# Yukun-Huang/DreamWaltz-G

Hardware: AMD Instinct MI355X
Metric: SDS steps/sec @512^2, 100k Gaussians, SD1.5+ControlNet; raster Mpix/s vs HBM roofline (higher is better)
Workload: dtype f32x

## Files before the change

dreamwaltz-g_amd/csrc/gemm.hip:

```cpp
#include "dwg_common.h"
#include "dwg_prof_internal.h"
#include "../../include/dwg_gemm.h"
#include <cstdlib>
#include <type_traits>

#if defined(DWG_GEMM_X_TU)
#include "dwg_xfmt.h"
typedef _Float16 HT;
#define DWG_DTYPE_HALF DWG_DTYPE_F32X
#define DWG_MFMA16(a, b, c) __builtin_amdgcn_mfma_f32_32x32x16_f16(a, b, c, 0, 0, 0)
#define DWG_HALF_NAME "f32x"
#elif defined(DWG_GEMM_F16_TU)
typedef _Float16 HT;
#define DWG_DTYPE_HALF DWG_DTYPE_F16
#define DWG_MFMA16(a, b, c) __builtin_amdgcn_mfma_f32_32x32x16_f16(a, b, c, 0, 0, 0)
#define DWG_HALF_NAME "f16"
#else
typedef __bf16 HT;
#define DWG_DTYPE_HALF DWG_DTYPE_BF16
#define DWG_MFMA16(a, b, c) __builtin_amdgcn_mfma_f32_32x32x16_bf16(a, b, c, 0, 0, 0)
#define DWG_HALF_NAME "bf16"
#endif

namespace {

typedef __attribute__((ext_vector_type(8))) HT bf16x8;
typedef __attribute__((ext_vector_type(16))) float f32x16;

struct ConvP {
    int enabled, Cin, Hin, Win, Hout, Wout, KH, KW, stride, pad_t, pad_l, dil;
    int up;
    int cin1;
    const void* A2;
};

struct GemmP {
    const void* A; const void* B; void* C; const void* bias; const void* residual;
    int M, N, K;
    long long sam, sak, sbn, sbk, ldc, ldr;
    int nb2;
    long long bA1, bA2, bB1, bB2, bC1, bC2, bR1, bR2;
    int act; float alpha;
    int out_bf16, res_bf16, bias_per_row, splitk, accumulate;
    float* ws;
    int bias_row_div;
    long long bias_ld;
    ConvP conv;
};

__device__ __forceinline__ float bf2f(HT x) { return (float)x; }
__device__ __forceinline__ HT f2bf(float x) { return (HT)x; }

struct bf16x4_t { HT v[4]; };
#ifdef DWG_GEMM_X_TU
__device__ __forceinline__ float ld_half1(const void* base, long long i) { return dwg_x_get1(base, i); }
__device__ __forceinline__ void st_half1(void* base, long long i, float v) { dwg_x_put1(base, i, v); }
__device__ __forceinline__ void ld_half4(const void* base, long long i, float (&v)[4]) { dwg_x_get4(base, i, v); }
__device__ __forceinline__ void st_half4(void* base, long long i, const float (&v)[4]) { dwg_x_put4(base, i, v); }
#else
__device__ __forceinline__ float ld_half1(const void* base, long long i) { return bf2f(reinterpret_cast<const HT*>(base)[i]); }
__device__ __forceinline__ void st_half1(void* base, long long i, float v) { reinterpret_cast<HT*>(base)[i] = f2bf(v); }
__device__ __forceinline__ void ld_half4(const void* base, long long i, float (&v)[4]) {
    const bf16x4_t r = *reinterpret_cast<const bf16x4_t*>(reinterpret_cast<const HT*>(base) + i);
#pragma unroll
    for (int e = 0; e < 4; e++) v[e] = bf2f(r.v[e]);
}
__device__ __forceinline__ void st_half4(void* base, long long i, const float (&v)[4]) {
    bf16x4_t o;
#pragma unroll
    for (int e = 0; e < 4; e++) o.v[e] = f2bf(v[e]);
    *reinterpret_cast<bf16x4_t*>(reinterpret_cast<HT*>(base) + i) = o;
}
#endif

template <bool LIGHT = false>
__device__ __forceinline__ float apply_act(float v, int act) {
    if constexpr (LIGHT) return act == 3 ? v / (1.f + __expf(-v)) : v;
    switch (act) {
        case 1: return v > 0.f ? v : 0.f;
        case 2: return v > 0.f ? v : 0.01f * v;
        case 3: return v / (1.f + __expf(-v));
        case 4: return 0.5f * v * (1.f + erff(v * 0.70710678118654752f));
        case 5: return 1.f / (1.f + __expf(-v));
        default: return v;
    }
}

// ... 840 lines not shown
    double f = 2.0 * p.M * p.N * p.K * batch;
#ifdef DWG_GEMM_X_TU
    f *= 0.5;
#endif
    if (p.conv.enabled && p.conv.dil > 1) f /= (double)(p.conv.dil * p.conv.dil);
    return f;
}

template <int BN, int AKIND>
static void launch_glds(const GemmP& p, int batch, hipStream_t stream, const char* name) {
    constexpr int S = (BN == 64 && AKIND != 1) ? 3 : 2;
    size_t lds = (size_t)S * (128 + BN) * 128;
    static bool attr_set = false;
    if (!attr_set) {
        hipFuncSetAttribute(reinterpret_cast<const void*>(&k_gemm_glds<BN, AKIND, S>), hipFuncAttributeMaxDynamicSharedMemorySize, (int)lds);
        attr_set = true;
    }
    dim3 grid(((p.M + 127) / 128) * ((p.N + BN - 1) / BN) * (p.splitk > 1 ? p.splitk : 1), 1, batch);
    static const char* const sym[2][4] = {{"k_gemm_glds<64, 0, 3>", "k_gemm_glds<64, 1, 2>", "k_gemm_glds<64, 2, 3>", "k_gemm_glds<64, 3, 3>"},
                                          {"k_gemm_glds<128, 0, 2>", "k_gemm_glds<128, 1, 2>", "k_gemm_glds<128, 2, 2>", "k_gemm_glds<128, 3, 2>"}};
    DWG_LAUNCH_W(name, sym[BN == 128][AKIND], gemm_flops(p, batch), (k_gemm_glds<BN, AKIND, S>), grid, dim3(256), lds, stream, p);
    launch_splitk_epilogue(p, stream);
}

template <int BM, int BN, int AKIND>
static void launch_glds8(const GemmP& p, int batch, hipStream_t stream, const char* name) {
    constexpr int S = 3;
    const size_t lds = (size_t)S * (BM + BN) * 128;
    static bool attr_set = false;
    if (!attr_set) {
        hipFuncSetAttribute(reinterpret_cast<const void*>(&k_gemm_glds8<BM, BN, AKIND, S>), hipFuncAttributeMaxDynamicSharedMemorySize, (int)lds);
        attr_set = true;
    }
    dim3 grid(((p.M + BM - 1) / BM) * ((p.N + BN - 1) / BN) * (p.splitk > 1 ? p.splitk : 1), 1, batch);
    static const char* const sym[2][4] = {
        {"k_gemm_glds8<256, 128, 0, 3>", "k_gemm_glds8<256, 128, 1, 3>", "k_gemm_glds8<256, 128, 2, 3>", "k_gemm_glds8<256, 128, 3, 3>"},
        {"k_gemm_glds8<128, 256, 0, 3>", "k_gemm_glds8<128, 256, 1, 3>", "k_gemm_glds8<128, 256, 2, 3>", "k_gemm_glds8<128, 256, 3, 3>"}};
    DWG_LAUNCH_W(name, sym[BN == 256][AKIND], gemm_flops(p, batch), (k_gemm_glds8<BM, BN, AKIND, S>), grid, dim3(512), lds, stream, p);
    launch_splitk_epilogue(p, stream);
}

template <bool V> struct BoolC { static constexpr bool value = V; };
template <int BN, int NW> struct Patch2Geom {
    static constexpr int PH = NW == 8 ? 16 : 8, PW = 16, HP = PH + 2, WP = PW + 2, NPIX = HP * WP, BM = PH * PW;
    static constexpr int NPI = (NPIX + 7) / 8;
    static constexpr int PPW = (NPI + NW - 1) / NW;
    static constexpr int WN = BN / 64, WM = NW / WN, TM = BM / WM / 32, TN = 2, NT = NW * 64;
    static constexpr int NJW = BN / (8 * NW);
    static constexpr int PBYTES = NPI * 8 * 128, BBYTES = BN * 128;
};

template <int BN, bool SPLIT, int NW, int NBS>
__global__ __launch_bounds__(NW * 64, 2) void k_conv3x3_patch2(GemmP p) {
    typedef Patch2Geom<BN, NW> G;
    constexpr int PH = G::PH, PW = G::PW, WP = G::WP, NPIX = G::NPIX, NPI = G::NPI, PPW = G::PPW;
    constexpr int WN = G::WN, WM = G::WM, TM = G::TM, TN = G::TN, NT = G::NT, NJW = G::NJW, BM = G::BM;
    constexpr int PBYTES = G::PBYTES, BBYTES = G::BBYTES;
    static_assert(NJW >= 1 && (NJW % 2 == 0 || NJW == 1), "row-block parity");
    extern __shared__ __attribute__((aligned(16))) unsigned char smem_raw[];
    unsigned char* sP = smem_raw;
    unsigned char* sB = smem_raw + 2 * PBYTES;
    const ConvP& cv = p.conv;
    const int tid = threadIdx.x, lane = tid & 63, wave = tid >> 6;
    const int wv = __builtin_amdgcn_readfirstlane(wave);
    const int wm = wave / WN, wn = wave % WN;
    const int tiles_x = (cv.Wout + PW - 1) / PW, tiles_y = (cv.Hout + PH - 1) / PH;
    const int nimg = p.M / (cv.Hout * cv.Wout);
    const int gm = nimg * tiles_y * tiles_x, ntn = (p.N + BN - 1) / BN;
    int id = blockIdx.x;
    {
        const int nwg = gridDim.x, q = nwg / 8, r = nwg % 8, xcd = id % 8, loc = id / 8;
        id = (xcd < r ? xcd * (q + 1) : r * (q + 1) + (xcd - r) * q) + loc;
    }
    int ks_id = 0;
    if constexpr (SPLIT) { ks_id = id / (gm * ntn); id -= ks_id * gm * ntn; }
    const int mt = id / ntn, n0 = (id % ntn) * BN;
    const int img = mt / (tiles_y * tiles_x), trem = mt % (tiles_y * tiles_x);
    const int y0 = (trem / tiles_x) * PH, x0 = (trem % tiles_x) * PW;
    const HT* X = reinterpret_cast<const HT*>(p.A) + (long long)img * cv.Hin * cv.Win * cv.Cin;
    const HT* Wt = reinterpret_cast<const HT*>(p.B);
    const HT* zero = reinterpret_cast<const HT*>(g_zero16);
    const int sub = lane >> 3, lg0 = (lane & 7) ^ (sub >> 1);

    auto issue_patch = [&](int cc, bool valid, unsigned char* dst) {
#pragma unroll
        for (int q = 0; q < PPW; q++) {
            int inst = wv + q * NW;
            if (inst >= NPI) inst -= NW;
            const int pi = inst * 8 + sub;
            const int py = pi / WP, px = pi - py * WP;
            const int iy = y0 - 1 + py, ix = x0 - 1 + px;
            const bool ok = valid && pi < NPIX && iy >= 0 && iy < cv.Hin && ix >= 0 && ix < cv.Win;
            const HT* src = ok ? X + ((long long)iy * cv.Win + ix) * cv.Cin + (lg0 ^ ((inst & 1) << 2)) * 8 + cc * 64 : zero;
            __builtin_amdgcn_global_load_lds((const __attribute__((address_space(1))) void*)src,
                                             (__attribute__((address_space(3))) void*)(dst + inst * 8 * 128), 16, 0, 0);
        }
    };
    const HT* wrow[NJW];
#pragma unroll
    for (int j = 0; j < NJW; j++) {
        const int r = n0 + (wv * NJW + j) * 8 + sub;
        wrow[j] = r < p.N ? Wt + (long long)r * p.sbn + (lg0 ^ (((wv * NJW + j) & 1) << 2)) * 8 : nullptr;
    }
    auto issue_w = [&](int cc, int tap, bool valid, unsigned char* dst) {
        const long long kofs = (long long)tap * cv.Cin + cc * 64;
#pragma unroll
        for (int j = 0; j < NJW; j++) {
            const HT* src = (valid && wrow[j]) ? wrow[j] + kofs : zero;
            __builtin_amdgcn_global_load_lds((const __attribute__((address_space(1))) void*)src,
                                             (__attribute__((address_space(3))) void*)(dst + (wv * NJW + j) * 8 * 128), 16, 0, 0);
        }
    };
    f32x16 acc[TM][TN];
#pragma unroll
    for (int i = 0; i < TM; i++)
#pragma unroll
        for (int j = 0; j < TN; j++)
#pragma unroll
            for (int r = 0; r < 16; r++) acc[i][j][r] = 0.f;
#ifdef DWG_GEMM_X_TU
    f32x16 acx[TM][TN];
#pragma unroll
    for (int i = 0; i < TM; i++)
#pragma unroll
        for (int j = 0; j < TN; j++)
#pragma unroll
            for (int r = 0; r < 16; r++) acx[i][j][r] = 0.f;
    constexpr int KS = 2, MPS = 3 * TM * TN;
    struct Frag { bf16x8 ah[TM], al[TM], bh[TN], bl[TN]; };
#else
    constexpr int KS = 4, MPS = TM * TN;
    struct Frag { bf16x8 af[TM], bf[TN]; };
#endif
    int pbase[TM];
#pragma unroll
    for (int i = 0; i < TM; i++) {
        const int r = (wm * TM + i) * 32 + (lane & 31);
        pbase[i] = (r / PW) * WP + (r % PW);
    }
    int cc0 = 0, ncc = cv.Cin / 64;
    if constexpr (SPLIT) {
        const int per = (ncc + p.splitk - 1) / p.splitk;
        cc0 = ks_id * per; ncc = min(ncc, cc0 + per);
    }
    const int frow = lane & 31, fx = (lane >> 1) & 7, fh = lane >> 5;
    const int nsteps = max(0, ncc - cc0) * 9;
    auto load_frags = [&](const unsigned char* pa, int toff, const unsigned char* tbs, int ks, Frag& f) {
        const unsigned char* tb = tbs + (wn * 64 + frow) * 128;
#ifdef DWG_GEMM_X_TU
        const int cl = ks * 4 + fh * 2;
#pragma unroll
        for (int i = 0; i < TM; i++) {
            const int pi = pbase[i] + toff, sw = (pi >> 1) & 7;
            f.ah[i] = *reinterpret_cast<const bf16x8*>(pa + pi * 128 + ((cl ^ sw) << 4));
            f.al[i] = *reinterpret_cast<const bf16x8*>(pa + pi * 128 + (((cl + 1) ^ sw) << 4));
        }
#pragma unroll
        for (int j = 0; j < TN; j++) {
            f.bh[j] = *reinterpret_cast<const bf16x8*>(tb + j * 32 * 128 + ((cl ^ fx) << 4));
            f.bl[j] = *reinterpret_cast<const bf16x8*>(tb + j * 32 * 128 + (((cl + 1) ^ fx) << 4));
        }
#else
        const int cl = ks * 2 + fh;
#pragma unroll
        for (int i = 0; i < TM; i++) {
            const int pi = pbase[i] + toff;
            f.af[i] = *reinterpret_cast<const bf16x8*>(pa + pi * 128 + ((cl ^ ((pi >> 1) & 7)) << 4));
        }
#pragma unroll
        for (int j = 0; j < TN; j++) f.bf[j] = *reinterpret_cast<const bf16x8*>(tb + j * 32 * 128 + ((cl ^ fx) << 4));
#endif
    };
    auto mma = [&](const Frag& f) {
#ifdef DWG_GEMM_X_TU
#pragma unroll
        for (int i = 0; i < TM; i++)
// ... 144 lines not shown
}
template <typename T, int BN>
static void dispatch_a(const GemmP& p, int amode, int bmode, int batch, hipStream_t s, const char* name) {
    if (amode == MODE_KVEC) dispatch_b<T, BN, MODE_KVEC>(p, bmode, batch, s, name);
    else if (amode == MODE_RVEC) dispatch_b<T, BN, MODE_RVEC>(p, bmode, batch, s, name);
    else if (amode == MODE_CONV) dispatch_b<T, BN, MODE_CONV>(p, bmode, batch, s, name);
    else dispatch_b<T, BN, MODE_SCALAR>(p, bmode, batch, s, name);
}

static int batch_of(const dwg_gemm_desc* d) { return d->batch1 * d->batch2; }

static int tile_bn(const dwg_gemm_desc* d) {
    if (d->N <= 64) return 64;
    const long long blocks128 = (long long)((d->M + 127) / 128) * ((d->N + 127) / 128) * batch_of(d);
    return blocks128 < 256 ? 64 : 128;
}

constexpr int kCUs = 256, kMinWgs = 200;
static bool fills_cus(long long wgs) {
    const long long rounds = (wgs + kCUs - 1) / kCUs;
    return wgs >= kMinWgs && wgs * 100 >= rounds * kCUs * 80;
}

constexpr int kSplitkTarget = 256;
constexpr int kSplitkNoSplit = 384;
constexpr int kSplitkMinSteps = 12;
static int auto_splitk(int M, int N, int K, int bn, int bk) {
    long long blocks = (long long)((M + 127) / 128) * ((N + bn - 1) / bn);
    if (blocks >= kSplitkNoSplit || K < 2 * kSplitkMinSteps * bk) return 1;
    if (2.0 * M * N * K < 4.0e8) return 1;
    long long sk = kSplitkTarget / blocks;
    long long kmax = K / (kSplitkMinSteps * bk);
    if (sk > kmax) sk = kmax;
    if (sk > 16) sk = 16;
    return sk >= 2 ? (int)sk : 1;
}

constexpr int kBigMinK = 1280, kBigMaxTiles = 2048;
constexpr int kBigMinSteps = 8, kBigSkMax = 24;
static int big_tile(int M, int N, int K, int* splitk_out) {
    *splitk_out = 1;
    if (K < kBigMinK) return 0;
    int bm = 0;
    if (M >= 192) { if (N >= 128 && (N % 128 == 0 || N >= 640)) bm = 256; }
    else if (N >= 256) bm = 128;
    if (!bm) return 0;
    const int bn = bm == 256 ? 128 : 256;
    const long long tiles = (long long)((M + bm - 1) / bm) * ((N + bn - 1) / bn);
    if (tiles > kBigMaxTiles) return 0;
    long long sk = 1;
    if (tiles < kCUs) {
        sk = kCUs / tiles;
        const long long kmax = K / (kBigMinSteps * 64);
        if (sk > kmax) sk = kmax;
        if (sk > kBigSkMax) sk = kBigSkMax;
        if (sk < 1) sk = 1;
    }
    if (!fills_cus(tiles * sk)) return 0;
    *splitk_out = (int)sk;
    return bm;
}

template <typename T>
static int pick_mode(const void* base, long long srow, long long sk, int nrows, int K, const long long* boffs, int nboffs) {
    constexpr int VEC = TT<T>::VEC;
    bool aligned = ((uintptr_t)base % 16) == 0;
    for (int i = 0; i < nboffs; i++) aligned = aligned && (boffs[i] % VEC == 0);
    if (sk == 1 && aligned && K % VEC == 0 && srow % VEC == 0) return MODE_KVEC;
    if (srow == 1 && aligned && nrows % VEC == 0 && sk % VEC == 0) return MODE_RVEC;
    return MODE_SCALAR;
}

static int splitk_of(const dwg_gemm_desc* d) {
    if (d->splitk > 1) return d->splitk;
    if (d->splitk != 0 || d->act == DWG_ACT_GEGLU_PAIR) return 1;
    return auto_splitk(d->M, d->N, d->K, tile_bn(d), d->dtype == DWG_DTYPE_HALF ? TT<HT>::BK : TT<float>::BK);
}
static bool slabs_possible(const dwg_gemm_desc* d) { return batch_of(d) == 1 && (long long)d->M * d->N < (1LL << 33); }
static long long fit_workspace(const dwg_gemm_desc* d, long long sk) {
    while (sk > 1 && (size_t)sk * d->M * d->N * sizeof(float) > d->workspace_bytes) sk--;
    return sk;
}

enum Family { FAM_GENERIC, FAM_GLDS, FAM_GLDS8, FAM_PATCH2 };
struct Plan {
    Family fam;
    int bm, bn, nw;
    int amode, bmode;
    int akind;
    int splitk;
    bool slabs;
};

constexpr int kPatchMinM = 8192;
constexpr int kPatch8MinSteps = 100;

static int make_plan(const dwg_gemm_desc* d, const GemmP& p, Plan& pl) {
    const bool half = d->dtype == DWG_DTYPE_HALF;
#if defined(DWG_GEMM_F16_TU) || defined(DWG_GEMM_X_TU)
    if (!half) return DWG_E_ARG;
#endif
    pl = Plan{FAM_GENERIC, 128, tile_bn(d), 4, MODE_KVEC, MODE_KVEC, 0, d->splitk > 1 ? d->splitk : 1, false};
    if (d->workspace && slabs_possible(d)) {
        pl.splitk = (int)fit_workspace(d, splitk_of(d));
        pl.slabs = pl.splitk > 1;
    }
    const long long ao[2] = {p.bA1, p.bA2}, bo[2] = {p.bB1, p.bB2};
    if (p.conv.enabled) {
        const int vec = half ? TT<HT>::VEC : TT<float>::VEC;
        if (d->conv_cin % vec != 0 || ((uintptr_t)d->A % 16) != 0) return DWG_E_ARG;
        if (d->A2 && (d->conv_cin1 % vec != 0 || d->conv_cin1 <= 0 || d->conv_cin1 >= d->conv_cin || ((uintptr_t)d->A2 % 16) != 0))
            return DWG_E_ARG;
        if (d->K != d->conv_kh * d->conv_kw * d->conv_cin) return DWG_E_ARG;
        pl.amode = MODE_CONV;
    } else {
        pl.amode = half ? pick_mode<HT>(p.A, p.sam, p.sak, p.M, p.K, ao, 2) : pick_mode<float>(p.A, p.sam, p.sak, p.M, p.K, ao, 2);
    }
    pl.bmode = half ? pick_mode<HT>(p.B, p.sbn, p.sbk, p.N, p.K, bo, 2) : pick_mode<float>(p.B, p.sbn, p.sbk, p.N, p.K, bo, 2);
    if (!half) return DWG_OK;
    if (pl.bmode != MODE_KVEC || (pl.amode != MODE_KVEC && pl.amode != MODE_CONV)) {
#ifdef DWG_GEMM_X_TU
        return DWG_E_ARG;
#else
        return DWG_OK;
#endif
    }
    const ConvP& cv = p.conv;
    const char* minm = getenv("DWG_CONV_PATCH_MINM");
    const int patch_min_m = minm ? atoi(minm) : kPatchMinM;
    const bool patch_geom = pl.amode == MODE_CONV && batch_of(d) == 1 && d->conv_kh == 3 && d->conv_kw == 3 && d->conv_stride == 1 &&
                            cv.dil == 1 && cv.up == 1 && d->conv_pad_t == 1 && d->conv_pad_l == 1 && !d->A2 && d->conv_cin % 64 == 0 &&
                            d->conv_hout == d->conv_hin && d->conv_wout == d->conv_win && d->conv_wout >= 16 && d->conv_hout >= 8;
    const int ncc = d->conv_cin / 64;
    if (patch_geom && d->splitk <= 1 && d->conv_hout % 16 == 0 && d->conv_wout % 16 == 0 && (d->N % 128 == 0 || d->N >= 512)) {
        const long long tiles8 = (long long)(d->M / 256) * ((d->N + 127) / 128);
        long long sk = 1;
        if (tiles8 < kMinWgs && d->workspace && d->splitk == 0 && slabs_possible(d)) {
            sk = kCUs / tiles8;
            if (sk > ncc / 2) sk = ncc / 2;
            sk = fit_workspace(d, sk);
            if (sk < 1) sk = 1;
            const long long per = (ncc + sk - 1) / sk;
            sk = (ncc + per - 1) / per;
        }
        const long long steps = (ncc + sk - 1) / sk * 9;
        const bool worth = sk > 1 || steps >= kPatch8MinSteps || d->M < patch_min_m;
        if (worth && fills_cus(tiles8 * sk) && (d->act == 0 || d->act == 3 || sk > 1)) {
            pl = Plan{FAM_PATCH2, 256, 128, 8, MODE_CONV, pl.bmode, 0, (int)sk, sk > 1};
            return DWG_OK;
        }
    }
    if (patch_geom && d->M >= patch_min_m && (d->act == 0 || d->act == 3 || pl.splitk > 1)) {
        if (pl.splitk > 1) {
            const int gm = (d->M / (d->conv_hout * d->conv_wout)) * ((d->conv_hout + 7) / 8) * ((d->conv_wout + 15) / 16);
            const int blocks = gm * ((d->N + pl.bn - 1) / pl.bn);
            int sk = blocks >= 256 ? 1 : (384 + blocks - 1) / blocks;
            if (sk > ncc / 2) sk = ncc / 2;
            if (sk > pl.splitk) sk = pl.splitk;
            if (sk < 2) sk = 1;
            pl.splitk = sk;
            pl.slabs = pl.slabs && sk > 1;
        }
        pl.fam = FAM_PATCH2;
        return DWG_OK;
    }
    const bool fast_geom = pl.amode == MODE_CONV && d->conv_cin % 64 == 0 && cv.dil == 1 && cv.up == 1 && d->conv_kh * d->conv_kw <= 32;
    const bool cat_fast = d->A2 && d->conv_cin1 % 64 == 0 && (d->conv_cin - d->conv_cin1) % 64 == 0;
    pl.akind = pl.amode != MODE_CONV ? 0 : (fast_geom && !d->A2 ? 2 : (fast_geom && cat_fast ? 3 : 1));
    int big_sk = 1;
    const int big_bm = d->splitk <= 1 ? big_tile(d->M, d->N, d->K, &big_sk) : 0;
    if (big_bm) {
        if (d->act == DWG_ACT_GEGLU_PAIR || !d->workspace || !slabs_possible(d) || d->splitk == 1) big_sk = 1;
        big_sk = (int)fit_workspace(d, big_sk);
        const int bbn = big_bm == 256 ? 128 : 256;
        const long long tiles = (long long)((d->M + big_bm - 1) / big_bm) * ((d->N + bbn - 1) / bbn) * batch_of(d);
        if (fills_cus(tiles * big_sk)) {
            pl = Plan{FAM_GLDS8, big_bm, bbn, 8, pl.amode, pl.bmode, pl.akind, big_sk, big_sk > 1};
            return DWG_OK;
        }
    }
    pl.fam = FAM_GLDS;
    return DWG_OK;
}

template <typename T>
static void launch_generic(const GemmP& p, const Plan& pl, int batch, hipStream_t s, const char* name) {
    if (pl.bn == 64) dispatch_a<T, 64>(p, pl.amode, pl.bmode, batch, s, name);
    else dispatch_a<T, 128>(p, pl.amode, pl.bmode, batch, s, name);
}
template <typename F>
static void with_akind(int akind, F f) {
    if (akind == 3) f(std::integral_constant<int, 3>{});
    else if (akind == 2) f(std::integral_constant<int, 2>{});
    else if (akind == 1) f(std::integral_constant<int, 1>{});
    else f(std::integral_constant<int, 0>{});
}

}

#ifdef DWG_GEMM_X_TU
static bool x_physical(const dwg_gemm_desc* d, dwg_gemm_desc* o) {
    if (!d) return false;
    *o = *d;
    if (d->dtype != DWG_DTYPE_F32X) return false;
    if (d->K % 8 || d->a_k_stride != 1 || d->b_k_stride != 1) return false;
    if ((d->a_row_stride | d->b_row_stride | d->a_batch1_stride | d->a_batch2_stride | d->b_batch1_stride | d->b_batch2_stride) % 8) return false;
    if (d->out_dtype == DWG_DTYPE_F32X && ((d->ldc | d->c_batch1_stride | d->c_batch2_stride) % 8 || ((uintptr_t)d->C % 16))) return false;
    if (d->residual && d->residual_dtype == DWG_DTYPE_F32X &&
        (((d->ldr ? d->ldr : d->ldc) | d->r_batch1_stride | d->r_batch2_stride) % 8 || ((uintptr_t)d->residual % 16))) return false;
    if (d->act == DWG_ACT_GEGLU_PAIR && d->out_dtype == DWG_DTYPE_F32X && d->N % 16) return false;
    if (d->conv_enabled && (d->conv_cin % 8 || (d->A2 && d->conv_cin1 % 8))) return false;
    o->K = 2 * d->K;
    o->a_row_stride = 2 * d->a_row_stride; o->b_row_stride = 2 * d->b_row_stride;
    o->a_batch1_stride = 2 * d->a_batch1_stride; o->a_batch2_stride = 2 * d->a_batch2_stride;
    o->b_batch1_stride = 2 * d->b_batch1_stride; o->b_batch2_stride = 2 * d->b_batch2_stride;
// ... 24 lines not shown
    if (d && d->dtype == DWG_DTYPE_F16) return dwg_gemm_workspace_bytes_f16(d);
    if (d && d->dtype == DWG_DTYPE_F32X) return dwg_gemm_workspace_bytes_x(d);
#endif
#ifdef DWG_GEMM_X_TU
    dwg_gemm_desc xd;
    if (!x_physical(d, &xd)) return 0;
    d = &xd;
#endif
    if (!d || d->M <= 0 || d->N <= 0 || !slabs_possible(d)) return 0;
    int sk = splitk_of(d);
    if (d->dtype == DWG_DTYPE_HALF && d->splitk == 0 && d->act != DWG_ACT_GEGLU_PAIR) {
        int bsk = 1;
        if (big_tile(d->M, d->N, d->K, &bsk) && bsk > sk) sk = bsk;
    }
    return sk > 1 ? (size_t)sk * d->M * d->N * sizeof(float) : 0;
}

int DWG_GEMM_FN(const dwg_gemm_desc* d, dwg_stream_t stream_) {
#if !defined(DWG_GEMM_F16_TU) && !defined(DWG_GEMM_X_TU)
    if (d && d->dtype == DWG_DTYPE_F16) return dwg_gemm_f16(d, stream_);
    if (d && d->dtype == DWG_DTYPE_F32X) return dwg_gemm_x(d, stream_);
#endif
#ifdef DWG_GEMM_X_TU
    dwg_gemm_desc xd;
    if (!x_physical(d, &xd)) return DWG_E_ARG;
    d = &xd;
#endif
    if (!d || !d->A || !d->B || !d->C) return DWG_E_ARG;
    if (d->M < 0 || d->N < 0 || d->K < 0 || d->batch1 < 1 || d->batch2 < 1) return DWG_E_ARG;
    if (d->M == 0 || d->N == 0) return DWG_OK;
    if (d->dtype != DWG_DTYPE_F32 && d->dtype != DWG_DTYPE_HALF) return DWG_E_ARG;
    if (d->splitk > 1 && !d->workspace && (d->out_dtype != DWG_DTYPE_F32 || d->bias || d->residual || d->act)) return DWG_E_ARG;
    if (d->accumulate && d->out_dtype != DWG_DTYPE_F32) return DWG_E_ARG;
    if (d->act == DWG_ACT_GEGLU_PAIR && (d->N % 64 != 0 || d->residual || d->splitk > 1 || d->bias_per_row || d->bias_row_div)) return DWG_E_ARG;
    if ((uintptr_t)d->workspace & 15) return DWG_E_ARG;
    GemmP p;
    p.A = d->A; p.B = d->B; p.C = d->C; p.bias = d->bias; p.residual = d->residual;
    p.M = d->M; p.N = d->N; p.K = d->K;
    p.sam = d->a_row_stride; p.sak = d->a_k_stride; p.sbn = d->b_row_stride; p.sbk = d->b_k_stride;
    p.ldc = d->ldc; p.ldr = d->ldr ? d->ldr : d->ldc;
    p.nb2 = d->batch2;
    p.bA1 = d->a_batch1_stride; p.bA2 = d->a_batch2_stride; p.bB1 = d->b_batch1_stride; p.bB2 = d->b_batch2_stride;
    p.bC1 = d->c_batch1_stride; p.bC2 = d->c_batch2_stride; p.bR1 = d->r_batch1_stride; p.bR2 = d->r_batch2_stride;
    p.act = d->act; p.alpha = d->alpha;
    p.out_bf16 = d->out_dtype == DWG_DTYPE_HALF; p.res_bf16 = d->residual_dtype == DWG_DTYPE_HALF;
    p.bias_per_row = d->bias_per_row; p.accumulate = d->accumulate;
    const bool plain1x1 = d->conv_enabled && d->conv_kh == 1 && d->conv_kw == 1 && d->conv_stride == 1 && d->conv_pad_t == 0 &&
                          d->conv_pad_l == 0 && d->conv_in_dilation <= 1 && d->conv_in_upsample <= 1 && !d->A2 && d->conv_hout == d->conv_hin &&
                          d->conv_wout == d->conv_win && d->K == d->conv_cin && batch_of(d) == 1;
    if (plain1x1) { p.sam = d->conv_cin; p.sak = 1; }
    p.conv.enabled = d->conv_enabled && !plain1x1;
    p.conv.Cin = d->conv_cin; p.conv.Hin = d->conv_hin; p.conv.Win = d->conv_win; p.conv.Hout = d->conv_hout;
    p.conv.Wout = d->conv_wout; p.conv.KH = d->conv_kh; p.conv.KW = d->conv_kw; p.conv.stride = d->conv_stride;
    p.conv.pad_t = d->conv_pad_t; p.conv.pad_l = d->conv_pad_l; p.conv.dil = d->conv_in_dilation > 1 ? d->conv_in_dilation : 1;
    p.conv.up = d->conv_in_upsample > 1 ? d->conv_in_upsample : 1;
    p.conv.A2 = d->A2; p.conv.cin1 = d->A2 ? d->conv_cin1 : d->conv_cin;
    p.bias_row_div = d->bias_row_div; p.bias_ld = d->bias_ld > 0 ? d->bias_ld : d->N;
    Plan pl;
    const int rc = make_plan(d, p, pl);
    if (rc != DWG_OK) return rc;
    p.splitk = pl.splitk;
    p.ws = pl.slabs ? reinterpret_cast<float*>(d->workspace) : nullptr;
    const int batch = batch_of(d);
    hipStream_t stream = (hipStream_t)stream_;
    const char* name = d->name ? d->name : (d->conv_enabled ? "conv_igemm" : "gemm");
    switch (pl.fam) {
        case FAM_PATCH2:
            if (pl.nw == 8) launch_conv3x3_patch2<128, 8, 4>(p, stream, name);
            else if (pl.bn == 64) launch_conv3x3_patch2<64, 4, 4>(p, stream, name);
            else launch_conv3x3_patch2<128, 4, 2>(p, stream, name);
            break;
        case FAM_GLDS8:
            with_akind(pl.akind, [&](auto ak) {
                if (pl.bm == 256) launch_glds8<256, 128, decltype(ak)::value>(p, batch, stream, name);
                else launch_glds8<128, 256, decltype(ak)::value>(p, batch, stream, name);
            });
            break;
        case FAM_GLDS:
            with_akind(pl.akind, [&](auto ak) {
                if (pl.bn == 64) launch_glds<64, decltype(ak)::value>(p, batch, stream, name);
                else launch_glds<128, decltype(ak)::value>(p, batch, stream, name);
            });
            break;
        case FAM_GENERIC:
#if defined(DWG_GEMM_X_TU)
            return DWG_E_ARG;
#elif defined(DWG_GEMM_F16_TU)
            launch_generic<HT>(p, pl, batch, stream, name);
#else
            if (d->dtype == DWG_DTYPE_HALF) launch_generic<HT>(p, pl, batch, stream, name);
            else launch_generic<float>(p, pl, batch, stream, name);
#endif
            break;
    }
    DWG_RETURN_IF_LAUNCH_FAILED();
    return DWG_OK;
}

}
```

Baseline: 39.44.

## Add thin-channel conv3x3 kernels and fuse 2x upsample into patch conv

```diff
diff --git a/dreamwaltz-g_amd/csrc/conv_thin.h b/dreamwaltz-g_amd/csrc/conv_thin.h
--- /dev/null
+++ b/dreamwaltz-g_amd/csrc/conv_thin.h
@@ -0,0 +1,17 @@
+#pragma once
+#include <hip/hip_runtime.h>
+
+struct dwg_thin_conv {
+    const void* X;
+    const void* W;
+    void* C;
+    const float* bias;
+    int M, N, Cin, Hin, Win, Hout, Wout, stride;
+    long long w_row, ldc;
+    int act;
+    int out_f32;
+    float alpha;
+};
+
+void dwg_conv_thin_in_launch(const dwg_thin_conv& t, hipStream_t stream, const char* name);
+void dwg_conv_thin_out_launch(const dwg_thin_conv& t, hipStream_t stream, const char* name);
diff --git a/dreamwaltz-g_amd/csrc/conv_thin.hip b/dreamwaltz-g_amd/csrc/conv_thin.hip
--- /dev/null
+++ b/dreamwaltz-g_amd/csrc/conv_thin.hip
@@ -0,0 +1,267 @@
+#include "dwg_common.h"
+#include "dwg_prof_internal.h"
+#include "dwg_xfmt.h"
+#include "conv_thin.h"
+
+namespace {
+
+typedef __attribute__((ext_vector_type(16))) float f32x16;
+typedef __attribute__((ext_vector_type(4))) float f32x4;
+
+__device__ __forceinline__ dwg_h8 zero_h8() {
+    dwg_h8 z;
+#pragma unroll
+    for (int e = 0; e < 8; e++) z[e] = (_Float16)0.f;
+    return z;
+}
+
+template <int CIN>
+__global__ __launch_bounds__(256, CIN == 8 ? 3 : 2) void k_conv3x3_thin_in(dwg_thin_conv t) {
+    constexpr int GPT = CIN / 8, NG = 9 * GPT, NS = (NG + 1) / 2;
+    const int lane = threadIdx.x & 63, col = lane & 31, h = lane >> 5;
+    const int wave = __builtin_amdgcn_readfirstlane(threadIdx.x >> 6);
+    const int nct = (t.N + 31) / 32;
+    const int gw = blockIdx.x * 4 + wave;
+    const int ct = gw % nct, slot = gw / nct, nslots = (gridDim.x * 4) / nct;
+    if (slot >= nslots) return;
+    const int n0 = ct * 32;
+    const unsigned char* X = reinterpret_cast<const unsigned char*>(t.X);
+
+    dwg_h8 bh[NS], bl[NS];
+    {
+        const unsigned char* wr = reinterpret_cast<const unsigned char*>(t.W) + (long long)(n0 + col) * t.w_row * 4;
+#pragma unroll
+        for (int s = 0; s < NS; s++) {
+            const int q = 2 * s + h;
+            const bool ok = n0 + col < t.N && q < NG;
+            bh[s] = ok ? *reinterpret_cast<const dwg_h8*>(wr + q * 32) : zero_h8();
+            bl[s] = ok ? *reinterpret_cast<const dwg_h8*>(wr + q * 32 + 16) : zero_h8();
+        }
+    }
+    float bias[2][8];
+#pragma unroll
+    for (int g = 0; g < 2; g++)
+#pragma unroll
+        for (int e = 0; e < 8; e++) {
+            const int n = n0 + (2 * g + h) * 8 + e;
+            bias[g][e] = (t.bias && n < t.N) ? t.bias[n] : 0.f;
+        }
+
+    const int ntiles = (t.M + 31) / 32, hw = t.Hout * t.Wout;
+    dwg_h8 ah[NS], al[NS];
+    auto load_tile = [&](int tile) {
+        const int m = tile * 32 + col;
+        const bool mok = tile < ntiles && m < t.M;
+        const int img = m / hw, rem = m - img * hw, oy = rem / t.Wout, ox = rem - oy * t.Wout;
+        const int iy0 = oy * t.stride - 1, ix0 = ox * t.stride - 1;
+        const unsigned char* xi = X + (long long)img * t.Hin * t.Win * (CIN * 4);
+#pragma unroll
+        for (int s = 0; s < NS; s++) {
+            const int Q0 = 2 * s >= NG ? NG - 1 : 2 * s, Q1 = 2 * s + 1 >= NG ? NG - 1 : 2 * s + 1;
+            const int tap = h ? Q1 / GPT : Q0 / GPT, cg = h ? Q1 % GPT : Q0 % GPT;
+            const int ky = h ? (Q1 / GPT) / 3 : (Q0 / GPT) / 3, kx = tap - 3 * ky;
+            const int iy = iy0 + ky, ix = ix0 + kx;
+            const bool ok = mok && 2 * s + h < NG && iy >= 0 && iy < t.Hin && ix >= 0 && ix < t.Win;
+            const unsigned char* src = xi + ((long long)iy * t.Win + ix) * (CIN * 4) + cg * 32;
+            ah[s] = ok ? *reinterpret_cast<const dwg_h8*>(src) : zero_h8();
+            al[s] = ok ? *reinterpret_cast<const dwg_h8*>(src + 16) : zero_h8();
+        }
+    };
+
+    load_tile(slot);
+    for (int tile = slot; tile < ntiles; tile += nslots) {
+        f32x16 acc, acx;
+#pragma unroll
+        for (int r = 0; r < 16; r++) { acc[r] = 0.f; acx[r] = 0.f; }
+#pragma unroll
+        for (int s = 0; s < NS; s++) acc = __builtin_amdgcn_mfma_f32_32x32x16_f16(bh[s], ah[s], acc, 0, 0, 0);
+#pragma unroll
+        for (int s = 0; s < NS; s++) acx = __builtin_amdgcn_mfma_f32_32x32x16_f16(bl[s], ah[s], acx, 0, 0, 0);
+#pragma unroll
+        for (int s = 0; s < NS; s++) acx = __builtin_amdgcn_mfma_f32_32x32x16_f16(bh[s], al[s], acx, 0, 0, 0);
+#pragma unroll
+        for (int r = 0; r < 16; r++) acc[r] = fmaf(acx[r], DWG_X_LO_INV, acc[r]);
+        load_tile(tile + nslots);
+
+        const int m = tile * 32 + col;
+        unsigned char* crow = reinterpret_cast<unsigned char*>(t.C) + ((long long)m * t.ldc + n0) * 4;
+#pragma unroll
+        for (int g = 0; g < 2; g++) {
+            float v[8];
+#pragma unroll
+            for (int e = 0; e < 4; e++) {
+                const float mine = h ? acc[8 * g + 4 + e] : acc[8 * g + e];
+                const float send = h ? acc[8 * g + e] : acc[8 * g + 4 + e];
+                const float recv = __shfl_xor(send, 32, 64);
+                v[e] = h ? recv : mine;
+                v[4 + e] = h ? mine : recv;
+            }
+            const int n = n0 + (2 * g + h) * 8;
+#pragma unroll
+            for (int e = 0; e < 8; e++) {
+                float y = fmaf(v[e], t.alpha, bias[g][e]);
+                v[e] = t.act == 3 ? y / (1.f + __expf(-y)) : y;
+            }
+            if (m < t.M && n < t.N) {
+                unsigned char* dst = crow + (2 * g + h) * 32;
+                if (t.out_f32) {
+                    f32x4 a = {v[0], v[1], v[2], v[3]}, b = {v[4], v[5], v[6], v[7]};
+                    *reinterpret_cast<f32x4*>(dst) = a;
+                    *reinterpret_cast<f32x4*>(dst + 16) = b;
+                } else {
+                    dwg_x8 o;
+#pragma unroll
+                    for (int e = 0; e < 8; e++) o.set(e, v[e]);
+                    o.store(reinterpret_cast<dwg_xs*>(dst));
+                }
+            }
+        }
+    }
+}
+
+__global__ __launch_bounds__(256, 3) void k_conv3x3_thin_out(dwg_thin_conv t) {
+    __shared__ float red[3][8][64];
+    const int lane = threadIdx.x & 63, col = lane & 31, h = lane >> 5;
+    const int wave = __builtin_amdgcn_readfirstlane(threadIdx.x >> 6);
+    const int nkc = t.Cin / 16, nst = 9 * nkc;
+    const int hw = t.Hout * t.Wout, nitems = (t.M + 63) / 64;
+    const long long pixb = (long long)t.Cin * 4;
+    const unsigned char* X = reinterpret_cast<const unsigned char*>(t.X);
+    const unsigned char* wr = reinterpret_cast<const unsigned char*>(t.W) + (long long)col * t.w_row * 4 + h * 32;
+    const bool wok = col < t.N;
+    float bias[4];
+#pragma unroll
+    for (int e = 0; e < 4; e++) bias[e] = (t.bias && h * 4 + e < t.N) ? t.bias[h * 4 + e] : 0.f;
+
+    for (int item = blockIdx.x; item < nitems; item += gridDim.x) {
+        const unsigned char* xi[2];
+        int oy[2], ox[2];
+        bool mok[2];
+#pragma unroll
+        for (int pt = 0; pt < 2; pt++) {
+            const int m = item * 64 + pt * 32 + col;
+            mok[pt] = m < t.M;
+            const int img = m / hw, rem = m - img * hw;
+            oy[pt] = rem / t.Wout; ox[pt] = rem - oy[pt] * t.Wout;
+            xi[pt] = X + (long long)img * t.Hin * t.Win * pixb + h * 32;
+        }
+        struct Frag { dwg_h8 ah[2], al[2], bh, bl; };
+        auto issue = [&](int st, Frag& f) {
+            const bool valid = st < nst;
+            const int tap = st / nkc, kc = st - tap * nkc, ky = tap / 3, kx = tap - 3 * ky;
+#pragma unroll
+            for (int pt = 0; pt < 2; pt++) {
+                const int iy = oy[pt] + ky - 1, ix = ox[pt] + kx - 1;
+                const bool ok = valid && mok[pt] && iy >= 0 && iy < t.Hin && ix >= 0 && ix < t.Win;
+                const unsigned char* src = xi[pt] + ((long long)iy * t.Win + ix) * pixb + kc * 64;
+                f.ah[pt] = ok ? *reinterpret_cast<const dwg_h8*>(src) : zero_h8();
+                f.al[pt] = ok ? *reinterpret_cast<const dwg_h8*>(src + 16) : zero_h8();
+            }
+            const unsigned char* ws = wr + ((long long)tap * t.Cin + kc * 16) * 4;
+            f.bh = (valid && wok) ? *reinterpret_cast<const dwg_h8*>(ws) : zero_h8();
+            f.bl = (valid && wok) ? *reinterpret_cast<const dwg_h8*>(ws + 16) : zero_h8();
+        };
+        f32x16 acc[2], acx[2];
+#pragma unroll
+        for (int pt = 0; pt < 2; pt++)
+#pragma unroll
+            for (int r = 0; r < 16; r++) { acc[pt][r] = 0.f; acx[pt][r] = 0.f; }
+        auto mma = [&](const Frag& f) {
+#pragma unroll
+            for (int pt = 0; pt < 2; pt++) acc[pt] = __builtin_amdgcn_mfma_f32_32x32x16_f16(f.bh, f.ah[pt], acc[pt], 0, 0, 0);
+#pragma unroll
+            for (int pt = 0; pt < 2; pt++) acx[pt] = __builtin_amdgcn_mfma_f32_32x32x16_f16(f.bl, f.ah[pt], acx[pt], 0, 0, 0);
+#pragma unroll
+            for (int pt = 0; pt < 2; pt++) acx[pt] = __builtin_amdgcn_mfma_f32_32x32x16_f16(f.bh, f.al[pt], acx[pt], 0, 0, 0);
+        };
+        Frag f0, f1;
+        issue(wave, f0);
+        for (int st = wave; st < nst; st += 8) {
+            issue(st + 4, f1);
+            mma(f0);
+            issue(st + 8, f0);
+            mma(f1);
+        }
+        float v[8];
+#pragma unroll
+        for (int pt = 0; pt < 2; pt++)
+#pragma unroll
+            for (int e = 0; e < 4; e++) v[pt * 4 + e] = fmaf(acx[pt][e], DWG_X_LO_INV, acc[pt][e]);
+        if (wave > 0) {
+#pragma unroll
+            for (int i = 0; i < 8; i++) red[wave - 1][i][lane] = v[i];
+        }
+        __syncthreads();
+        if (wave == 0) {
+#pragma unroll
+            for (int w = 0; w < 3; w++)
+#pragma unroll
+                for (int i = 0; i < 8; i++) v[i] += red[w][i][lane];
+#pragma unroll
+            for (int pt = 0; pt < 2; pt++) {
+                const int m = item * 64 + pt * 32 + col;
+                float y[4];
+#pragma unroll
+                for (int e = 0; e < 4; e++) {
+                    const float z = fmaf(v[pt * 4 + e], t.alpha, bias[e]);
+                    y[e] = t.act == 3 ? z / (1.f + __expf(-z)) : z;
+                }
+                if (m < t.M) {
+                    if (t.out_f32) {
+                        float* dst = reinterpret_cast<float*>(t.C) + (long long)m * t.ldc + h * 4;
+                        if (t.N == 8 && (t.ldc & 3) == 0) {
+                            f32x4 o = {y[0], y[1], y[2], y[3]};
+                            *reinterpret_cast<f32x4*>(dst) = o;
+                        } else {
+#pragma unroll
+                            for (int e = 0; e < 4; e++)
+                                if (h * 4 + e < t.N) dst[e] = y[e];
+                        }
+                    } else {
+                        dwg_x_put4(reinterpret_cast<unsigned char*>(t.C) + (long long)m * t.ldc * 4, h * 4, y);
+                    }
+                }
+            }
+        }
+        __syncthreads();
+    }
+}
+
+}
+
+template <int CIN>
+static void launch_thin_in(const dwg_thin_conv& t, hipStream_t stream, const char* name, const char* sym) {
+    static int resident = 0;
+    if (!resident) {
+        int dev = 0, cus = 0, per_cu = 0;
+        (void)hipGetDevice(&dev);
+        (void)hipDeviceGetAttribute(&cus, hipDeviceAttributeMultiprocessorCount, dev);
+        (void)hipOccupancyMaxActiveBlocksPerMultiprocessor(&per_cu, reinterpret_cast<const void*>(&k_conv3x3_thin_in<CIN>), 256, 0);
+        resident = (cus > 0 ? cus : 256) * (per_cu > 0 ? per_cu : 2) * 4;
+    }
+    const long long nct = (t.N + 31) / 32, items = (long long)((t.M + 31) / 32) * nct;
+    long long waves = items < resident ? items : resident / nct * nct;
+    if (waves < nct) waves = nct;
+    const dim3 grid((unsigned)((waves + 3) / 4));
+    const double flops = 2.0 * t.M * t.N * 9.0 * t.Cin;
+    DWG_LAUNCH_W(name, sym, flops, (k_conv3x3_thin_in<CIN>), grid, dim3(256), 0, stream, t);
+}
+
+void dwg_conv_thin_in_launch(const dwg_thin_conv& t, hipStream_t stream, const char* name) {
+    if (t.Cin == 8) launch_thin_in<8>(t, stream, name, "k_conv3x3_thin_in<8>");
+    else launch_thin_in<16>(t, stream, name, "k_conv3x3_thin_in<16>");
+}
+
+void dwg_conv_thin_out_launch(const dwg_thin_conv& t, hipStream_t stream, const char* name) {
+    static int resident = 0;
+    if (!resident) {
+        int dev = 0, cus = 0, per_cu = 0;
+        (void)hipGetDevice(&dev);
+        (void)hipDeviceGetAttribute(&cus, hipDeviceAttributeMultiprocessorCount, dev);
+        (void)hipOccupancyMaxActiveBlocksPerMultiprocessor(&per_cu, reinterpret_cast<const void*>(&k_conv3x3_thin_out), 256, 0);
+        resident = (cus > 0 ? cus : 256) * (per_cu > 0 ? per_cu : 2);
+    }
+    const int nitems = (t.M + 63) / 64;
+    const dim3 grid((unsigned)(nitems < resident ? nitems : resident));
+    DWG_LAUNCH_W(name, "k_conv3x3_thin_out", 2.0 * t.M * t.N * 9.0 * t.Cin, k_conv3x3_thin_out, grid, dim3(256), 0, stream, t);
+}
diff --git a/dreamwaltz-g_amd/csrc/gemm.hip b/dreamwaltz-g_amd/csrc/gemm.hip
--- a/dreamwaltz-g_amd/csrc/gemm.hip
+++ b/dreamwaltz-g_amd/csrc/gemm.hip
@@ -3,6 +3,9 @@
 #include "../../include/dwg_gemm.h"
 #include <cstdlib>
 #include <type_traits>
+#ifdef DWG_GEMM_X_TU
+#include "conv_thin.h"
+#endif
 
 #if defined(DWG_GEMM_X_TU)
 #include "dwg_xfmt.h"
@@ -1009,6 +1012,7 @@
     const HT* zero = reinterpret_cast<const HT*>(g_zero16);
     const int sub = lane >> 3, lg0 = (lane & 7) ^ (sub >> 1);
 
+    const int ush = cv.up > 1 ? 1 : 0;
     auto issue_patch = [&](int cc, bool valid, unsigned char* dst) {
 #pragma unroll
         for (int q = 0; q < PPW; q++) {
@@ -1017,8 +1021,8 @@
             const int pi = inst * 8 + sub;
             const int py = pi / WP, px = pi - py * WP;
             const int iy = y0 - 1 + py, ix = x0 - 1 + px;
-            const bool ok = valid && pi < NPIX && iy >= 0 && iy < cv.Hin && ix >= 0 && ix < cv.Win;
-            const HT* src = ok ? X + ((long long)iy * cv.Win + ix) * cv.Cin + (lg0 ^ ((inst & 1) << 2)) * 8 + cc * 64 : zero;
+            const bool ok = valid && pi < NPIX && iy >= 0 && iy < cv.Hout && ix >= 0 && ix < cv.Wout;
+            const HT* src = ok ? X + ((long long)(iy >> ush) * cv.Win + (ix >> ush)) * cv.Cin + (lg0 ^ ((inst & 1) << 2)) * 8 + cc * 64 : zero;
             __builtin_amdgcn_global_load_lds((const __attribute__((address_space(1))) void*)src,
                                              (__attribute__((address_space(3))) void*)(dst + inst * 8 * 128), 16, 0, 0);
         }
@@ -1329,7 +1333,7 @@
     return sk;
 }
 
-enum Family { FAM_GENERIC, FAM_GLDS, FAM_GLDS8, FAM_PATCH2 };
+enum Family { FAM_GENERIC, FAM_GLDS, FAM_GLDS8, FAM_PATCH2, FAM_THIN_IN, FAM_THIN_OUT };
 struct Plan {
     Family fam;
     int bm, bn, nw;
@@ -1341,6 +1345,23 @@
 
 constexpr int kPatchMinM = 8192;
 constexpr int kPatch8MinSteps = 100;
+
+#ifdef DWG_GEMM_X_TU
+static bool thin_in_geom(const dwg_gemm_desc* d, const ConvP& cv) {
+    return batch_of(d) == 1 && d->conv_kh == 3 && d->conv_kw == 3 && (d->conv_stride == 1 || d->conv_stride == 2) && cv.dil == 1 && cv.up == 1 &&
+           d->conv_pad_t == 1 && d->conv_pad_l == 1 && !d->A2 && (d->conv_cin == 16 || d->conv_cin == 32) && d->N % 8 == 0 && !d->residual &&
+           !d->bias_per_row && !d->bias_row_div && (d->act == 0 || d->act == 3) && d->splitk <= 1 && !d->accumulate && d->ldc % 8 == 0 &&
+           ((uintptr_t)d->C % 16) == 0 && (d->out_dtype == DWG_DTYPE_F32 || d->out_dtype == DWG_DTYPE_F32X) &&
+           d->M == (d->M / (d->conv_hout * d->conv_wout)) * d->conv_hout * d->conv_wout;
+}
+static bool thin_out_geom(const dwg_gemm_desc* d, const ConvP& cv) {
+    return batch_of(d) == 1 && d->conv_kh == 3 && d->conv_kw == 3 && d->conv_stride == 1 && cv.dil == 1 && cv.up == 1 && d->conv_pad_t == 1 &&
+           d->conv_pad_l == 1 && !d->A2 && d->conv_cin % 64 == 0 && d->N <= 8 && d->conv_hout == d->conv_hin && d->conv_wout == d->conv_win &&
+           !d->residual && !d->bias_per_row && !d->bias_row_div && (d->act == 0 || d->act == 3) && d->splitk <= 1 && !d->accumulate &&
+           ((uintptr_t)d->C % 16) == 0 && (d->out_dtype == DWG_DTYPE_F32 || (d->out_dtype == DWG_DTYPE_F32X && d->N == 8 && d->ldc % 8 == 0)) &&
+           d->M == (d->M / (d->conv_hout * d->conv_wout)) * d->conv_hout * d->conv_wout;
+}
+#endif
 
 static int make_plan(const dwg_gemm_desc* d, const GemmP& p, Plan& pl) {
     const bool half = d->dtype == DWG_DTYPE_HALF;
@@ -1373,11 +1394,21 @@
 #endif
     }
     const ConvP& cv = p.conv;
+#ifdef DWG_GEMM_X_TU
+    if (pl.amode == MODE_CONV && thin_in_geom(d, cv)) {
+        pl.fam = FAM_THIN_IN; pl.splitk = 1; pl.slabs = false;
+        return DWG_OK;
+    }
+    if (pl.amode == MODE_CONV && thin_out_geom(d, cv)) {
+        pl.fam = FAM_THIN_OUT; pl.splitk = 1; pl.slabs = false;
+        return DWG_OK;
+    }
+#endif
     const char* minm = getenv("DWG_CONV_PATCH_MINM");
     const int patch_min_m = minm ? atoi(minm) : kPatchMinM;
     const bool patch_geom = pl.amode == MODE_CONV && batch_of(d) == 1 && d->conv_kh == 3 && d->conv_kw == 3 && d->conv_stride == 1 &&
-                            cv.dil == 1 && cv.up == 1 && d->conv_pad_t == 1 && d->conv_pad_l == 1 && !d->A2 && d->conv_cin % 64 == 0 &&
-                            d->conv_hout == d->conv_hin && d->conv_wout == d->conv_win && d->conv_wout >= 16 && d->conv_hout >= 8;
+                            cv.dil == 1 && cv.up <= 2 && d->conv_pad_t == 1 && d->conv_pad_l == 1 && !d->A2 && d->conv_cin % 64 == 0 &&
+                            d->conv_hout == cv.up * d->conv_hin && d->conv_wout == cv.up * d->conv_win && d->conv_wout >= 16 && d->conv_hout >= 8;
     const int ncc = d->conv_cin / 64;
     if (patch_geom && d->splitk <= 1 && d->conv_hout % 16 == 0 && d->conv_wout % 16 == 0 && (d->N % 128 == 0 || d->N >= 512)) {
         const long long tiles8 = (long long)(d->M / 256) * ((d->N + 127) / 128);
@@ -1568,6 +1599,18 @@
                 else launch_glds<128, decltype(ak)::value>(p, batch, stream, name);
             });
             break;
+        case FAM_THIN_IN:
+        case FAM_THIN_OUT: {
+#ifdef DWG_GEMM_X_TU
+            dwg_thin_conv t;
+            t.X = p.A; t.W = p.B; t.C = p.C; t.bias = reinterpret_cast<const float*>(p.bias);
+            t.M = p.M; t.N = p.N; t.Cin = p.conv.Cin / 2; t.Hin = p.conv.Hin; t.Win = p.conv.Win; t.Hout = p.conv.Hout; t.Wout = p.conv.Wout;
+            t.stride = p.conv.stride; t.w_row = p.sbn / 2; t.ldc = p.ldc; t.act = p.act; t.out_f32 = !p.out_bf16; t.alpha = p.alpha;
+            if (pl.fam == FAM_THIN_IN) dwg_conv_thin_in_launch(t, stream, name);
+            else dwg_conv_thin_out_launch(t, stream, name);
+#endif
+            break;
+        }
         case FAM_GENERIC:
 #if defined(DWG_GEMM_X_TU)
             return DWG_E_ARG;
```

After: 39.70 (median of 6 runs). No clear change (+0.6%).
